# acg-team/ProGraphMSA

Hardware: AMD Instinct MI355X
Metric: DP cell-updates/sec (GCUPS) + wall-clock on 256 seqs × 1000 aa, WAG (higher is better)
Workload: dtype f32

## Files before the change

include/pgm_hip.h:

```cpp
#ifndef PGM_HIP_H_
#define PGM_HIP_H_

#include <stdint.h>
#include <stddef.h>

#ifdef __cplusplus
extern "C" {
#endif

#define PGM_OK 0
#define PGM_ERR_INVALID 1
#define PGM_ERR_DEVICE 2
#define PGM_ERR_BACKTRACK 3
#define PGM_ERR_NOMEM 4

#define PGM_GAP 0xFFFFFFFFu


typedef struct pgm_graph {
    uint32_t n;
    uint32_t dim;
    const double *sites;
    const int32_t *e_rowptr;
    const uint32_t *e_col;
// ... 61 lines not shown
uint64_t pgm_align_batch_cells(const pgm_align_batch *b);
int pgm_align_batch_time(pgm_ctx *ctx, pgm_align_batch *b, int reps, float *ms_prep,
                         float *ms_emission, float *ms_fill, float *ms_traceback);
int pgm_align_batch_stage_times(pgm_align_batch *b, int reset, float *ms_prep, float *ms_emission, float *ms_fill,
                                uint32_t *launches);
int pgm_align_batch_job_times(pgm_ctx *ctx, pgm_align_batch *b, uint64_t *ticks);
int pgm_align_batch_test_stall(pgm_align_batch *b, uint32_t job, uint32_t band, uint32_t spin_limit);
int pgm_test_cu_shares(uint32_t cus, double lean_cost, uint32_t nlean, double band_cost, uint32_t nbands, double rest_cost,
                       uint32_t nrest, uint32_t ncrit, double longest_chain, uint32_t *out4);
#define PGM_PLAN_HEAD 23
#define PGM_PLAN_DHEAD 9
#define PGM_PLAN_JOB 19
int pgm_test_batch_plan(uint32_t njobs, const pgm_graph *const *g1, const pgm_graph *const *g2, const pgm_model *const *model,
                        const pgm_scores *scores, uint32_t flags, const pgm_site_ref *res1, const pgm_site_ref *res2, uint32_t cus,
                        uint32_t *head, double *dhead, uint32_t *job_fields, uint32_t *items, uint32_t *bands, uint32_t *lean_list, int32_t *tblist);
int pgm_align_batch_read_matrices(pgm_ctx *ctx, pgm_align_batch *b, uint32_t job, float *M,
                                  float *X, float *Y, float *W, float *S);

int pgm_nw_pairs_batch(pgm_ctx *ctx, uint32_t dim, const int32_t *score, int32_t gap_open,
                       int32_t gap_extend, uint32_t nseq, const int8_t *syms,
                       const uint32_t *offs, uint32_t npairs, const uint32_t *pi,
                       const uint32_t *pj, int32_t *counts, uint32_t *gaps);
#define PGM_NW_REDUCED 1u
int pgm_nw_pairs_submit(pgm_ctx *ctx, uint32_t dim, const int32_t *score, int32_t gap_open,
                        int32_t gap_extend, uint32_t nseq, const int8_t *syms,
                        const uint32_t *offs, uint32_t npairs, const uint32_t *pi,
                        const uint32_t *pj, uint32_t flags, int32_t *counts, uint32_t *gaps, int *ticket);
int pgm_nw_pairs_wait(pgm_ctx *ctx, int ticket);
float pgm_nw_last_kernel_ms(pgm_ctx *ctx);
void *pgm_host_alloc(size_t bytes);
// ... 144 lines not shown
```

prographmsa_amd/__init__.py:

```python
import ctypes as C
import os

_HERE = os.path.dirname(os.path.abspath(__file__))
LIB_PATH = os.path.join(_HERE, "lib", "libpgm_hip.so")
PGMSA_PATH = os.path.join(_HERE, "bin", "pgmsa")

PGM_OK, PGM_ERR_INVALID, PGM_ERR_DEVICE, PGM_ERR_BACKTRACK, PGM_ERR_NOMEM = 0, 1, 2, 3, 4
PGM_GAP = 0xFFFFFFFF
PGM_BATCH_KEEP_MATRICES = 1
PGM_NW_REDUCED = 1
PGM_MERGE_RESIDENT = 1


class pgm_graph(C.Structure):
    _fields_ = [("n", C.c_uint32), ("dim", C.c_uint32), ("sites", C.POINTER(C.c_double)),
                ("e_rowptr", C.POINTER(C.c_int32)), ("e_col", C.POINTER(C.c_uint32)), ("e_val", C.POINTER(C.c_float)),
                ("r_rowptr", C.POINTER(C.c_int32)), ("r_col", C.POINTER(C.c_uint32)), ("r_units", C.POINTER(C.c_uint32))]


class pgm_model(C.Structure):
    _fields_ = [("M", C.POINTER(C.c_double)), ("pi", C.POINTER(C.c_double))]


class pgm_scores(C.Structure):
# ... 34 lines not shown
    _fields_ = [("index1", C.c_uint32), ("index2", C.c_uint32), ("dist1", C.c_double), ("dist2", C.c_double)]


class pgm_bionj_pair(C.Structure):
    _fields_ = [("index1", C.c_uint32), ("index2", C.c_uint32)]


class pgm_align_out(C.Structure):
    _fields_ = [("score", C.c_float), ("n_tr_indels", C.c_uint32), ("len", C.c_uint32), ("status", C.c_int32),
                ("map1", C.POINTER(C.c_uint32)), ("map2", C.POINTER(C.c_uint32))]


EXPORTS = [
    "pgm_device_count", "pgm_ctx_create", "pgm_ctx_destroy", "pgm_last_error", "pgm_ctx_device_info",
    "pgm_align_graphs_batch", "pgm_align_batch_create", "pgm_align_batch_create_ex", "pgm_align_batch_create_res", "pgm_align_graphs_batch_res", "pgm_align_batch_run", "pgm_align_batch_fetch",
    "pgm_align_batch_destroy", "pgm_align_batch_cells", "pgm_align_batch_test_stall", "pgm_test_cu_shares", "pgm_test_batch_plan", "pgm_align_batch_stage_times", "pgm_align_batch_job_times", "pgm_align_batch_time", "pgm_align_batch_read_matrices",
    "pgm_nw_pairs_batch", "pgm_nw_pairs_submit", "pgm_nw_pairs_wait", "pgm_nw_last_kernel_ms", "pgm_host_alloc", "pgm_host_free", "pgm_csprofile_load", "pgm_csprofile_create_batch", "pgm_csprofile_create_batch_res",
    "pgm_csprofile_last_kernel_ms", "pgm_mldist_batch", "pgm_prealigned_counts_batch", "pgm_kmer_cosine", "pgm_dist_last_kernel_ms",
    "pgm_kmer_cosine_multi", "pgm_prealigned_counts_multi", "pgm_prealigned_counts_resampled",
    "pgm_merge_profiles_batch", "pgm_merge_profiles_batch_ex", "pgm_resident_reset", "pgm_resident_onehot", "pgm_resident_import", "pgm_merge_last_kernel_ms",
    "pgm_gapmask_extend_batch", "pgm_gap_parsimony_batch", "pgm_parsimony_last_kernel_ms",
    "pgm_wls_load", "pgm_wls_pair_sums_batch", "pgm_wls_last_kernel_ms", "pgm_wls_last_launches",
    "pgm_bionj", "pgm_bionj_multi", "pgm_bionj_last_launches", "pgm_bionj_last_kernel_ms",
    "pgm_bionj_plan", "pgm_bionj_plan_multi",
    "pgm_msa_agreement", "pgm_agreement_last_kernel_ms",
    "pgm_transfer_min", "pgm_transfer_last_kernel_ms", "pgm_transfer_taxa",
    "pgm_tree_likelihood", "pgm_treelik_last_kernel_ms", "pgm_tree_likelihood_rates", "pgm_tree_ancestral", "pgm_tree_nni",
    "pgm_resampled_sums", "pgm_resample_last_kernel_ms",
]


# ... 11 lines not shown
        "pgm_last_error": (C.c_char_p, []),
        "pgm_ctx_device_info": (C.c_int, [vp, C.c_char_p, C.c_size_t, C.POINTER(C.c_int)]),
        "pgm_align_graphs_batch": (C.c_int, [vp, u32, PG, PG, PM, C.POINTER(pgm_scores), C.POINTER(pgm_align_out)]),
        "pgm_align_batch_create": (C.c_int, [vp, u32, PG, PG, PM, C.POINTER(pgm_scores), C.POINTER(vp)]),
        "pgm_align_batch_create_ex": (C.c_int, [vp, u32, PG, PG, PM, C.POINTER(pgm_scores), u32, C.POINTER(vp)]),
        "pgm_align_batch_create_res": (C.c_int, [vp, u32, PG, PG, PM, C.POINTER(pgm_scores), u32, C.POINTER(pgm_site_ref), C.POINTER(pgm_site_ref), C.POINTER(vp)]),
        "pgm_align_graphs_batch_res": (C.c_int, [vp, u32, PG, PG, PM, C.POINTER(pgm_scores), C.POINTER(pgm_site_ref), C.POINTER(pgm_site_ref), C.POINTER(pgm_align_out)]),
        "pgm_align_batch_run": (C.c_int, [vp, vp]),
        "pgm_align_batch_fetch": (C.c_int, [vp, vp, C.POINTER(pgm_align_out)]),
        "pgm_align_batch_destroy": (None, [vp, vp]),
        "pgm_align_batch_cells": (C.c_uint64, [vp]),
        "pgm_align_batch_test_stall": (C.c_int, [vp, u32, u32, u32]),
        "pgm_test_cu_shares": (C.c_int, [u32, C.c_double, u32, C.c_double, u32, C.c_double, u32, u32, C.c_double, C.POINTER(C.c_uint32)]),
        "pgm_test_batch_plan": (C.c_int, [u32, PG, PG, PM, C.POINTER(pgm_scores), u32, C.POINTER(pgm_site_ref), C.POINTER(pgm_site_ref), u32,
                                          C.POINTER(u32), C.POINTER(C.c_double)] + [C.POINTER(u32)] * 4 + [C.POINTER(i32)]),
        "pgm_align_batch_stage_times": (C.c_int, [vp, C.c_int] + [C.POINTER(C.c_float)] * 3 + [C.POINTER(u32)]),
        "pgm_align_batch_job_times": (C.c_int, [vp, vp, C.POINTER(C.c_uint64)]),
        "pgm_align_batch_time": (C.c_int, [vp, vp, C.c_int] + [C.POINTER(C.c_float)] * 4),
        "pgm_align_batch_read_matrices": (C.c_int, [vp, vp, u32] + [C.POINTER(C.c_float)] * 5),
        "pgm_nw_pairs_batch": (C.c_int, [vp, u32, C.POINTER(i32), i32, i32, u32, C.POINTER(C.c_int8), C.POINTER(u32), u32,
                                         C.POINTER(u32), C.POINTER(u32), C.POINTER(i32), C.POINTER(u32)]),
        "pgm_nw_pairs_submit": (C.c_int, [vp, u32, C.POINTER(i32), i32, i32, u32, C.POINTER(C.c_int8), C.POINTER(u32), u32,
                                          C.POINTER(u32), C.POINTER(u32), u32, C.POINTER(i32), C.POINTER(u32), C.POINTER(C.c_int)]),
        "pgm_nw_pairs_wait": (C.c_int, [vp, C.c_int]),
        "pgm_host_alloc": (vp, [C.c_size_t]),
        "pgm_host_free": (None, [vp]),
        "pgm_nw_last_kernel_ms": (C.c_float, [vp]),
        "pgm_csprofile_load": (C.c_int, [vp, u32, u32] + [C.POINTER(C.c_double)] * 3),
        "pgm_csprofile_create_batch": (C.c_int, [vp, u32, C.POINTER(C.c_int8), C.POINTER(u32)] + [C.POINTER(C.c_double)] * 4
                                       + [C.POINTER(C.c_uint64)]),
# ... 253 lines not shown
```

prographmsa_amd/csrc/pgm_align_kernels.h:

```cpp
#ifndef PGM_ALIGN_KERNELS_H_
#define PGM_ALIGN_KERNELS_H_

#include <hip/hip_runtime.h>
#include <math.h>
#include <type_traits>
#include "pgm_device.h"

#define PGM_NEG_INF (-INFINITY)

__device__ __forceinline__ float pgm_ls_log_add(float x, float add) {
    const float a = 2.44247459618085927548717403238913328776812604856113966238617812902399112761292613763080658235564f;
    const float b = -4.2040783745848554315883301529007786406310628696382695994938550046831869207082846248658671f;
    const float c = -0.72123729809042963774358701619456664388406302428056983119308906451199556380646306f;
    const uint32_t bits = __float_as_uint(x);
    const float e = (float)((int32_t)(bits >> 23) - 126);
    const float d = __uint_as_float(((bits << 9) >> 9) ^ 0x3f000000u);
    float t = __fdiv_rn(b, __fsub_rn(d, c));
    const float u = __fadd_rn(e, a);
    t = __fadd_rn(t, add);
    t = __fadd_rn(t, u);
    return t;
}

__device__ __forceinline__ float pgm_emission_finish(float num, float ay, float bx, float match_init) {
    float q = __fdiv_rn(num, __fmul_rn(ay, bx));
    if (q != q) q = __uint_as_float(0xFFC00000u);
    return pgm_ls_log_add(q, match_init);
}

template <int DMAX, int NODES>
__global__ void __launch_bounds__(NODES) pgm_prep_kernel(const PgmJob *__restrict__ jobs, int *__restrict__ sync, uint32_t sync_ints) {
    extern __shared__ float prep_lds[];
    {
        const uint32_t nthreads = gridDim.x * gridDim.y * gridDim.z * NODES;
        const uint32_t gid = ((blockIdx.z * gridDim.y + blockIdx.y) * gridDim.x + blockIdx.x) * NODES + threadIdx.x;
        for (uint32_t i = gid; i < sync_ints; i += nthreads) sync[i] = 0;
    }
    const PgmJob &J = jobs[blockIdx.x];
    const bool first = blockIdx.y == 0;
    const uint32_t n = first ? J.n1 : J.n2;
    const uint32_t v0 = blockIdx.z * NODES;
    if (v0 >= n) return;
    if (J.tabhdr && J.tabhdr[0] == 0) {
        const uint32_t nc = J.dim + 2u;
        bool any = n - 1u >= v0 && n - 1u < v0 + (uint32_t)NODES;
        for (uint32_t c = 0; c < nc; ++c) {
            const uint32_t r = (uint32_t)J.tabhdr[1u + (first ? 0u : nc) + c];
            any = any || (r != 0u && r - 1u >= v0 && r - 1u < v0 + (uint32_t)NODES);
        }
        if (!any) return;
    }
    const uint32_t D = J.dim, DP = J.dp, ST = D + 1;
    float *Mf = prep_lds;
    float *pif = prep_lds + D * D;
    float *nl = pif + D;
    const uint32_t nn = min((uint32_t)NODES, n - v0);
    {
        const int32_t *pp = first ? J.pp1 : J.pp2;
        const uint32_t *pc = first ? J.pc1 : J.pc2, *pu = first ? J.pu1 : J.pu2;
        const float *pv = first ? J.pv1 : J.pv2;
        PgmTbNode *rec = (first ? J.tb1 : J.tb2) + v0;
        for (uint32_t i = threadIdx.x; i < nn * PGM_TB_PK; i += NODES) {
            const uint32_t node = i / PGM_TB_PK, k = i % PGM_TB_PK;
            const int32_t eb = pp[v0 + node];
            const uint32_t cnt = (uint32_t)(pp[v0 + node + 1] - eb);
            const int32_t e = cnt == 0u ? 0 : eb + (int32_t)min(k, cnt - 1u);
// ... 48 lines not shown
        for (uint32_t k = 0; k < D; ++k) {
            float t = 0.0f;
#pragma unroll
            for (int j = 0; j < DMAX; ++j)
                if ((uint32_t)j < D) t = __fadd_rn(t, __fmul_rn(Mf[j + D * k], g[j]));
            nl[v * ST + k] = t;
        }
    }
    __syncthreads();
    for (uint32_t i = threadIdx.x; i < nn * DP; i += NODES) {
        const uint32_t node = i / DP, k = i % DP;
        dst[i] = k < D ? nl[node * ST + k] : 0.0f;
    }
}

#define PGM_TAB_HDR 136
__global__ void __launch_bounds__(256) pgm_classify_kernel(const PgmJob *__restrict__ jobs) {
    const PgmJob &J = jobs[blockIdx.x];
    if (!J.tabhdr) return;
    const bool first = blockIdx.y == 0;
    const uint32_t n = first ? J.n1 : J.n2, D = J.dim;
    const double *sites = first ? J.sites1 : J.sites2;
    const uint32_t *smap = first ? J.smap1 : J.smap2;
    uint8_t *cls = (uint8_t *)(first ? J.cls1 : J.cls2);
    const float uni = (float)(1.0 / (double)D);
    for (uint32_t v = blockIdx.z * blockDim.x + threadIdx.x; v < n; v += gridDim.z * blockDim.x) {
        const double *col = sites + (size_t)D * (smap ? smap[v] : v);
        uint32_t nz = 0, sym = 0;
        bool same = true;
        float vs = 0.f;
        const float g0 = (float)col[0];
// ... 15 lines not shown
__device__ __forceinline__ size_t pgm_cell_index(const PgmJob &J, uint32_t y, uint32_t x) {
    const uint32_t b = y / PGM_ROWS, l = PGM_HALO + (y - b * PGM_ROWS);
    return ((size_t)b * J.tsteps + (x + l)) * 64u + l;
}
__device__ __forceinline__ float4 pgm_load_cell(const PgmJob &J, uint32_t y, uint32_t x) {
    return J.cells[pgm_cell_index(J, y, x)];
}

__device__ __forceinline__ float pgm_dpp_wave_shr1(float src, float lane0_value) {
    return __int_as_float(__builtin_amdgcn_update_dpp(__float_as_int(lane0_value), __float_as_int(src), 0x138, 0xf, 0xf, false));
}

#define PGM_GLOBAL __attribute__((address_space(1)))
typedef float pgm_v4f __attribute__((ext_vector_type(4)));
template <class T> __device__ __forceinline__ T pgm_gld(const T *p) { return *(const PGM_GLOBAL T *)(uintptr_t)p; }
#define PGM_EM_TB 4
template <int DP, int RB>
__global__ void __launch_bounds__(4 * PGM_ROWS) pgm_emission_skew_kernel(const PgmJob *__restrict__ jobs) {
    typedef float pgm_v2f __attribute__((ext_vector_type(2)));
    constexpr int NT = DP / 4;
    constexpr int COLS = 64 + PGM_EM_TB * PGM_BLOCK - PGM_HALO - 1;
    constexpr int STR = DP + 1;
    __shared__ pgm_v2f tp[(COLS + 1) * STR];
    __shared__ float bq[COLS];
    const PgmJob &J = jobs[blockIdx.z];
    const uint32_t tb0 = blockIdx.x * PGM_EM_TB;
    const uint32_t rsh = J.rshift, nvb = J.nb << rsh;
    if (tb0 >= J.nblk || 4u * RB * blockIdx.y >= nvb) return;
    if (J.tabhdr && pgm_gld(J.tabhdr) == 0) return;
    auto row_of = [&](uint32_t v, uint32_t lane_) { return ((((v >> rsh) << 6) + lane_) << rsh) | (v & ((1u << rsh) - 1u)); };
    auto sblock_of = [&](uint32_t v, uint32_t tb_) { return ((((size_t)(v >> rsh) * J.nblk + tb_) << rsh) | (v & ((1u << rsh) - 1u))); };
    const uint32_t t0 = tb0 * PGM_BLOCK;
    const int cbase = (int)t0 - 63;
    if ((DP == 20 || DP == 4) && RB == 1) {
        constexpr int TE = DP + 1;
        float *const tab = (float *)tp;
        static_assert(COLS * TE <= (COLS + 1) * STR * 2, "score table must fit the column staging area");
        static_assert(DP > 20 || TE <= 32, "row classes must fit As");
        __shared__ float As[32];
        const uint32_t fb0 = 4u * blockIdx.y + threadIdx.x / PGM_ROWS;
        const uint32_t fl = threadIdx.x % PGM_ROWS;
        const bool active = fb0 < nvb;
        int sym = DP;
        bool plain = true;
        float a_row = 0.f;
        if (active) {
            const uint32_t y = row_of(fb0, fl);
            const uint32_t yc = (y + 1 < J.n1) ? y : 0u;
            const float4 *src = (const float4 *)(J.g1f + (size_t)DP * yc);
            int nz = 0;
#pragma unroll
            for (int q = 0; q < NT; ++q) {
                const float4 v = src[q];
                const float vv[4] = {v.x, v.y, v.z, v.w};
#pragma unroll
// ... 48 lines not shown
        float4 v = make_float4(0.f, 0.f, 0.f, 0.f);
        if (c >= 0 && c <= (int)J.ncol) v = t2q[(size_t)NT * c + q];
        const float vv[4] = {v.x, v.y, v.z, v.w};
#pragma unroll
        for (int u = 0; u < 4; ++u) {
            const int k = 4 * q + u;
            if (ci < COLS) tpf[2 * (ci * STR + k)] = vv[u];
            if (ci > 0) tpf[2 * ((ci - 1) * STR + k) + 1] = vv[u];
        }
    }
    for (int i = threadIdx.x; i < COLS; i += 4 * PGM_ROWS) {
        const int col = cbase + i;
        bq[i] = (col >= 0 && col <= (int)J.ncol) ? J.b2[col] : 0.f;
    }
    __syncthreads();
    const uint32_t b0 = (4u * blockIdx.y + threadIdx.x / PGM_ROWS) * RB;
    const int l = PGM_HALO + (int)(threadIdx.x % PGM_ROWS);
    if (b0 >= nvb) return;
    float gy[RB][DP], ay[RB];
#pragma unroll
    for (int r = 0; r < RB; ++r) {
        const uint32_t y = row_of(b0 + (uint32_t)r, (uint32_t)(l - PGM_HALO));
        const uint32_t yc = (y + 1 < J.n1) ? y : 0u;
        const float4 *src = (const float4 *)(J.g1f + (size_t)DP * yc);
#pragma unroll
        for (int q = 0; q < NT; ++q) {
            const float4 v = src[q];
            gy[r][4 * q] = v.x; gy[r][4 * q + 1] = v.y; gy[r][4 * q + 2] = v.z; gy[r][4 * q + 3] = v.w;
        }
        ay[r] = J.a1[yc];
    }
// ... 2301 lines not shown
```

prographmsa_amd/csrc/pgm_capi.hip:

```cpp
#include <hip/hip_runtime.h>

#include <algorithm>
#include <cmath>
#include <cstdio>
#include <thread>
#include <atomic>
#include <chrono>
#include <queue>
#include <cstdlib>
#include <cstring>
#include <numeric>
#include <mutex>
#include <string>
#include <unordered_set>
#include <vector>
#include <sys/mman.h>

#include "pgm_align_kernels.h"
#include "pgm_crit_kernels.h"
#include "pgm_nw_kernels.h"
#include "pgm_csprofile_kernels.h"
#include "pgm_dist_kernels.h"
#include "pgm_merge_kernels.h"
#include "pgm_parsimony_kernels.h"
// ... 137 lines not shown
    size_t in_bytes = 0, work_bytes = 0, cell_bytes = 0, out_bytes = 0, s_bytes = 0, small_bytes = 0;
    size_t cap[8] = {0, 0, 0, 0, 0, 0, 0, 0};
    uint8_t *h_out = nullptr;
    uint8_t *h_in = nullptr;
    int *h_flag = nullptr;
    int *d_sync = nullptr;
    size_t sync_ints = 0;
    uint32_t lq_off = 0;
    PgmJob *d_jobs = nullptr;
    uint32_t *d_order = nullptr;
    PgmItem *d_items = nullptr;
    uint32_t *d_lean = nullptr;
    PgmItem *d_bands = nullptr;
    int2 *d_tblist = nullptr;
    unsigned long long *d_times = nullptr;
    int *d_tabhdr = nullptr;
    hipEvent_t ev_fork = nullptr, ev_join = nullptr;
    hipEvent_t ev_join_b = nullptr, ev_join_c = nullptr;
    uint32_t test_spin_limit = 0, test_stall_job = 0xFFFFFFFFu, test_stall_band = 0;
    double acc_ms[3] = {0, 0, 0};
    uint32_t acc_n = 0;
    bool ev_pending = false;
    std::vector<size_t> res_off, map1_off, map2_off;
    hipEvent_t ev[5] = {nullptr, nullptr, nullptr, nullptr, nullptr};
};
static const struct BatchBuffer { int slot; size_t reserve_mb; uint8_t *pgm_align_batch::*ptr; size_t pgm_align_batch::*bytes; } kBatchBuffers[6] = {
    {pgm_ctx::C_IN, 128, &pgm_align_batch::d_in, &pgm_align_batch::in_bytes}, {pgm_ctx::C_WORK, 256, &pgm_align_batch::d_work, &pgm_align_batch::work_bytes},
    {pgm_ctx::C_CELLS, 2048, &pgm_align_batch::d_cells, &pgm_align_batch::cell_bytes}, {pgm_ctx::C_OUT, 8, &pgm_align_batch::d_out, &pgm_align_batch::out_bytes},
    {pgm_ctx::C_S, 1024, &pgm_align_batch::d_S, &pgm_align_batch::s_bytes}, {pgm_ctx::C_SMALL, 4, &pgm_align_batch::d_small, &pgm_align_batch::small_bytes}};

// ... 228 lines not shown
}

#define PGM_STATUS_PENDING 0x7ffffff0
struct PrepTier { uint32_t tier, threads; size_t lds; };
static PrepTier prep_tier(uint32_t maxdim) {
    const uint32_t tier = alphabet_tier(maxdim), threads = tier == 64u ? 64u : 256u;
    return {tier, threads, ((size_t)maxdim * maxdim + maxdim + threads * ((size_t)maxdim + 1)) * sizeof(float)};
}
static hipError_t launch_all(pgm_ctx *ctx, pgm_align_batch *b, bool timed) {
    hipStream_t s = ctx->stream;
    const BatchSchedule &S = b->sched;
    hipError_t e;
    for (uint32_t i = 0; i < b->njobs; ++i) ((PgmJob::Result *)(b->h_out + b->res_off[i]))->status = PGM_STATUS_PENDING;
    if (timed && (e = hipEventRecord(b->ev[0], s)) != hipSuccess) return e;
    const PrepTier T = prep_tier(b->maxdim);
    const dim3 pg(b->njobs, 2, (b->maxn + T.threads - 1) / T.threads);
    if (T.tier == 4) hipLaunchKernelGGL((pgm_prep_kernel<4, 256>), pg, dim3(256), T.lds, s, b->d_jobs, b->d_sync, (uint32_t)b->sync_ints);
    else if (T.tier == 20) hipLaunchKernelGGL((pgm_prep_kernel<20, 256>), pg, dim3(256), T.lds, s, b->d_jobs, b->d_sync, (uint32_t)b->sync_ints);
    else hipLaunchKernelGGL((pgm_prep_kernel<64, 64>), pg, dim3(64), T.lds, s, b->d_jobs, b->d_sync, (uint32_t)b->sync_ints);
    if ((e = hipGetLastError()) != hipSuccess) return e;
    if (timed && (e = hipEventRecord(b->ev[1], s)) != hipSuccess) return e;
    const dim3 eg((b->maxnblk + PGM_EM_TB - 1) / PGM_EM_TB, (b->maxnb + 3) / 4, b->njobs);
    if (T.tier == 4) hipLaunchKernelGGL((pgm_emission_skew_kernel<4, 1>), eg, dim3(4 * PGM_ROWS), 0, s, b->d_jobs);
    else if (T.tier == 20) hipLaunchKernelGGL((pgm_emission_skew_kernel<20, 1>), eg, dim3(4 * PGM_ROWS), 0, s, b->d_jobs);
    else hipLaunchKernelGGL((pgm_emission_skew_kernel<64, 1>), eg, dim3(4 * PGM_ROWS), 0, s, b->d_jobs);
    if ((e = hipGetLastError()) != hipSuccess) return e;
    if (timed && (e = hipEventRecord(b->ev[2], s)) != hipSuccess) return e;
    const uint32_t spin_limit = b->test_spin_limit ? b->test_spin_limit : PGM_SPIN_LIMIT, stall_job = b->test_stall_job, stall_band = b->test_stall_band;
    const bool fork = S.nlean != 0;
    const bool bandk = S.nbands != 0;
    const bool tbk = (S.nitems != 0 || bandk) && (S.ntb + S.ntb_c + S.ntb_b) != 0;
    const bool critk = S.ncrit != 0;
    if ((fork || bandk || critk) && (e = hipEventRecord(b->ev_fork, s)) != hipSuccess) return e;
    if (critk && (e = hipStreamWaitEvent(ctx->stream4, b->ev_fork, 0)) != hipSuccess) return e;
    if (fork && (e = hipStreamWaitEvent(ctx->stream2, b->ev_fork, 0)) != hipSuccess) return e;
    if (bandk && (e = hipStreamWaitEvent(ctx->stream3, b->ev_fork, 0)) != hipSuccess) return e;
    const uint32_t nrest = S.nitems - S.ncrit;
    hipStream_t sc = critk ? s : ctx->stream4, sr = critk ? ctx->stream4 : s;
    auto sweep = [&](hipStream_t st, uint32_t workers, const PgmItem *list, uint32_t n, bool c3, uint32_t ticket_off) {
        if (c3) hipLaunchKernelGGL(pgm_crit_kernel, dim3(workers), dim3(64 * PGM_C3_WAVES), 0, st, b->d_jobs, list, n, b->d_sync, spin_limit, stall_job, stall_band, ticket_off);
// ... 21 lines not shown
        if (tbk && S.ntb_c) tracebacks(sc, S.ncrit_workers, S.ntb, S.ntb_c, b->lq_off + 2 * njp, 16u);
        if ((e = hipGetLastError()) != hipSuccess) return e;
    }
    if (tbk && S.ntb) {
        tracebacks(sr, S.ntb_workers, 0u, S.ntb, b->lq_off, 0u);
        if ((e = hipGetLastError()) != hipSuccess) return e;
    }
    if (critk && (e = hipEventRecord(b->ev_join_c, ctx->stream4)) != hipSuccess) return e;
    if (bandk && (e = hipStreamWaitEvent(s, b->ev_join_b, 0)) != hipSuccess) return e;
    if (critk && (e = hipStreamWaitEvent(s, b->ev_join_c, 0)) != hipSuccess) return e;
    if (fork && ((e = hipEventRecord(b->ev_join, ctx->stream2)) != hipSuccess || (e = hipStreamWaitEvent(s, b->ev_join, 0)) != hipSuccess)) return e;
    if (timed && (e = hipEventRecord(b->ev[3], s)) != hipSuccess) return e;
    if (timed && (e = hipEventRecord(b->ev[4], s)) != hipSuccess) return e;
    return hipSuccess;
}
struct SmallLayout { size_t sync, jobs, order, items, lean, tblist, bands, times, tabhdr, total_bands; bool any_lean; };
static SmallLayout layout_small(pgm_align_batch *b) {
    SmallLayout s;
    const uint32_t njobs = b->njobs;
    s.total_bands = 0; s.any_lean = false;
    for (const PgmJob &J : b->jobs) { s.total_bands += J.nb; s.any_lean = s.any_lean || (J.lean && !J.keep_cells); }
    DevLayout SM;
    s.sync = SM.take(b->sync_ints * sizeof(int)); s.jobs = SM.take(sizeof(PgmJob) * std::max(1u, njobs));
    s.order = SM.take(4 * (size_t)std::max(1u, njobs)); s.items = SM.take(sizeof(PgmItem) * std::max<size_t>(1, s.total_bands));
    s.lean = SM.take(4 * (size_t)std::max(1u, njobs)); s.tblist = SM.take(8 * (size_t)std::max(1u, njobs));
    s.bands = SM.take(sizeof(PgmItem) * std::max<size_t>(1, s.total_bands)); s.times = SM.take(16 * (size_t)std::max(1u, njobs) + 16);
    s.tabhdr = SM.take(s.any_lean ? 4 * (size_t)PGM_TAB_HDR * njobs : 16);
    b->small_bytes = SM.bytes;
    return s;
}

static double now_ms() { return std::chrono::duration<double, std::milli>(std::chrono::steady_clock::now().time_since_epoch()).count(); }

struct BatchAlloc {
    std::atomic<int> state{0};
    hipError_t err = hipSuccess, host_err = hipSuccess;
    uint8_t *h_out_dev = nullptr;
    double ms_dev = 0, ms_host = 0, ms_slot[6] = {0, 0, 0, 0, 0, 0};
};
static void take_batch_buffers(pgm_ctx *ctx, pgm_align_batch *b, SmallLayout sm, BatchAlloc *A) {
    const double ta0 = now_ms();
    hipError_t e2 = hipSetDevice(ctx->device);
// ... 1 lines not shown
    for (int k = 0; k < 6 && e2 == hipSuccess; ++k) {
        const BatchBuffer &s = kBatchBuffers[k];
        e2 = cache_take(ctx, s.slot, b->*s.bytes, (void **)&(b->*s.ptr), &b->cap[s.slot]);
        const double t = now_ms(); A->ms_slot[k] = t - tprev; tprev = t;
    }
    if (e2 == hipSuccess) {
        b->d_sync = (int *)(b->d_small + sm.sync);
        b->d_jobs = (PgmJob *)(b->d_small + sm.jobs);
        b->d_order = (uint32_t *)(b->d_small + sm.order);
        b->d_items = (PgmItem *)(b->d_small + sm.items);
        b->d_lean = (uint32_t *)(b->d_small + sm.lean);
        b->d_tblist = (int2 *)(b->d_small + sm.tblist);
        b->d_bands = (PgmItem *)(b->d_small + sm.bands);
        b->d_times = (unsigned long long *)(b->d_small + sm.times);
        b->d_tabhdr = sm.any_lean ? (int *)(b->d_small + sm.tabhdr) : nullptr;
    }
    A->err = e2;
    A->state.store(e2 == hipSuccess ? 1 : -1, std::memory_order_release);
    A->ms_dev = now_ms() - ta0;
    if (e2 == hipSuccess) {
        hipError_t e3 = cache_take(ctx, pgm_ctx::C_HOST, b->out_bytes + 64, (void **)&b->h_out, &b->cap[pgm_ctx::C_HOST]);
        if (e3 == hipSuccess) b->h_flag = (int *)(b->h_out + (b->out_bytes + 15) / 16 * 16);
        if (e3 == hipSuccess) e3 = hipHostGetDevicePointer((void **)&A->h_out_dev, b->h_out, 0);
        A->host_err = e3;
    }
    A->ms_host = now_ms() - ta0 - A->ms_dev;
}

struct CreateGuard {
    pgm_ctx *ctx;
// ... 80 lines not shown
                                       S.nworkers, S.nlean_workers, S.nband_workers, S.nwide_workers, S.ncrit_workers, S.ntb_workers, S.ntb_b_workers,
                                       S.crit_c3, S.rest_c3, S.capacity, (uint32_t)S.total_b, (uint32_t)S.total, (uint32_t)S.total_c};
    const double d[PGM_PLAN_DHEAD] = {S.rsweep, S.t_goal, S.lean_cost, S.band_cost, S.band_end, S.other_cost, S.fill_end, S.crit_end, Z.pro.longest_crit_chain};
    memcpy(head, h, sizeof h);
    memcpy(dhead, d, sizeof d);
    for (uint32_t i = 0; i < njobs; ++i) {
        const PgmJob &J = jobs[i];
        const uint32_t f[PGM_PLAN_JOB] = {J.lean, J.has_extras, J.mode2, J.hD, J.hDX, J.slot_bytes, J.aux_off, J.ov_off, J.rh_off, J.c3_off, J.nov2, J.has_far, J.long1, J.long2,
                                          J.crit3, J.far_slack, J.nslots, Z.off[i].s1.ngeneric + Z.off[i].s2.ngeneric, Z.off[i].s1.nkill + Z.off[i].s2.nkill};
        memcpy(job_fields + (size_t)PGM_PLAN_JOB * i, f, sizeof f);
    }
    if (S.nitems) memcpy(items, S.items.data(), sizeof(PgmItem) * S.nitems);
    if (S.nbands) memcpy(bands, S.bands.data(), sizeof(PgmItem) * S.nbands);
    if (S.nlean) memcpy(lean_list, S.lean_list.data(), 4 * (size_t)S.nlean);
    if (S.ntb + S.ntb_c + S.ntb_b) memcpy(tblist, S.tblist.data(), 8 * (size_t)(S.ntb + S.ntb_c + S.ntb_b));
    return PGM_OK;
}

int pgm_align_batch_create(pgm_ctx *ctx, uint32_t njobs, const pgm_graph *const *g1, const pgm_graph *const *g2,
                           const pgm_model *const *model, const pgm_scores *scores, pgm_align_batch **out) {
    return pgm_align_batch_create_ex(ctx, njobs, g1, g2, model, scores, 0u, out);
}

int pgm_align_batch_create_ex(pgm_ctx *ctx, uint32_t njobs, const pgm_graph *const *g1, const pgm_graph *const *g2,
                              const pgm_model *const *model, const pgm_scores *scores, uint32_t flags, pgm_align_batch **out) {
    return pgm_align_batch_create_res(ctx, njobs, g1, g2, model, scores, flags, nullptr, nullptr, out);
}

int pgm_align_batch_create_res(pgm_ctx *ctx, uint32_t njobs, const pgm_graph *const *g1, const pgm_graph *const *g2,
                               const pgm_model *const *model, const pgm_scores *scores, uint32_t flags,
// ... 59 lines not shown
    b->order = size_order(b->jobs);
    b->sched = plan_schedule(b->jobs, b->order, cus);
    const BatchSchedule &S = b->sched;
    if (cprof && njobs)
        fprintf(stderr, "    work lists: longest chain of sweeps %.0f us, goal %.0f us; lean %zu jobs %.0f us-worker on %u CUs; bands %zu, %.0f us-worker on %u CUs (simulated end %.0f us); items %zu, %.0f us-worker on %u CUs (simulated end %.0f us), of the longest chains %zu on %u CUs (%.0f us)\n",
                S.rsweep, S.t_goal, (size_t)S.nlean, S.lean_cost, S.nlean_workers, S.total_b, S.band_cost, S.nband_workers, S.band_end, S.total, S.other_cost, S.capacity, S.fill_end, S.total_c, S.ncrit_workers, S.crit_end);
    const double tc4 = now_ms();
    if (S.nitems > std::max<size_t>(1, sm.total_bands)) return fail(PGM_ERR_DEVICE, "work list longer than the number of bands");
    if ((e = (hipError_t)upload_err.load()) != hipSuccess ||
        (e = hipMemcpyAsync(b->d_tblist, S.tblist.data(), 8 * S.tblist.size(), hipMemcpyHostToDevice, ctx->stream)) != hipSuccess ||
        (e = hipMemcpyAsync(b->d_jobs, b->jobs.data(), sizeof(PgmJob) * njobs, hipMemcpyHostToDevice, ctx->stream)) != hipSuccess ||
        (e = hipMemcpyAsync(b->d_order, b->order.data(), 4 * (size_t)njobs, hipMemcpyHostToDevice, ctx->stream)) != hipSuccess ||
        (e = hipMemcpyAsync(b->d_items, S.items.data(), sizeof(PgmItem) * S.items.size(), hipMemcpyHostToDevice, ctx->stream)) != hipSuccess ||
        (e = hipMemcpyAsync(b->d_lean, S.lean_list.data(), 4 * S.lean_list.size(), hipMemcpyHostToDevice, ctx->stream)) != hipSuccess ||
        (e = hipMemcpyAsync(b->d_bands, S.bands.data(), sizeof(PgmItem) * S.bands.size(), hipMemcpyHostToDevice, ctx->stream)) != hipSuccess ||
        (e = classify_lean_jobs(ctx, b)) != hipSuccess ||
        (e = hipStreamSynchronize(ctx->stream)) != hipSuccess)
        return fail(PGM_ERR_DEVICE, std::string("upload: ") + hipGetErrorString(e));
    for (int k = 0; k < 5; ++k) (void)hipEventCreate(&b->ev[k]);
    (void)hipEventCreateWithFlags(&b->ev_fork, hipEventDisableTiming);
    (void)hipEventCreateWithFlags(&b->ev_join, hipEventDisableTiming);
    (void)hipEventCreateWithFlags(&b->ev_join_b, hipEventDisableTiming);
    (void)hipEventCreateWithFlags(&b->ev_join_c, hipEventDisableTiming);
    if (cprof)
        fprintf(stderr, "    create: sizes %.2f ms, pinned input block %.2f, flatten %.2f, wait for the allocations %.2f (device %.2f, pinned results %.2f), work list %.2f, upload of %.1f MB %.2f\n",
                tc0 - tcs, tc1 - tc0, tc2 - tc1, tc3 - tc2, A.ms_dev, A.ms_host, tc4 - tc3, b->in_bytes / 1e6, now_ms() - tc4);
    if (cprof)
        fprintf(stderr, "    device buffers: inputs %.1f MB %.2f ms, work %.1f MB %.2f, cells %.1f MB %.2f, results %.1f MB %.2f, S %.1f MB %.2f, small %.2f\n",
                b->in_bytes / 1e6, A.ms_slot[0], b->work_bytes / 1e6, A.ms_slot[1], b->cell_bytes / 1e6, A.ms_slot[2], b->out_bytes / 1e6, A.ms_slot[3], b->s_bytes / 1e6, A.ms_slot[4], A.ms_slot[5]);
    *out = G.release();
    return PGM_OK;
// ... 235 lines not shown
```

prographmsa_amd/csrc/pgm_device.h:

```cpp
#ifndef PGM_DEVICE_H_
#define PGM_DEVICE_H_

#include <stdint.h>
#include "../../include/pgm_hip.h"

#define PGM_MAX_DIM 64
#define PGM_HALO 0
#define PGM_ROWS 64
#define PGM_VL 16
#define PGM_BLOCK 8
#define PGM_NRING 128
#define PGM_KF 4
#define PGM_KF8 8
#define PGM_DCAP 28
#define PGM_PF 4
#define PGM_REMOTE_MAX 128
#define PGM_WAVES 8
#define PGM_WIDE_WAVES 4
#define PGM_POOL 163584
#define PGM_CPARTS 3
#define PGM_AUX_RES 0
#define PGM_AUX_SBLK 3072
#define PGM_AUX_EL 9216
#define PGM_AUX_CNT 13312
// ... 109 lines not shown
#define PGM_LK_H 16u
#define PGM_LK_TAB (3u * PGM_LK_T * PGM_LK_T)
__host__ __device__ inline uint32_t pgm_lk_first(uint32_t n1, uint32_t n2, uint32_t lcols, uint32_t r) {
    const uint32_t w = lcols < PGM_LK_W ? lcols : PGM_LK_W;
    const uint64_t xc = ((uint64_t)(PGM_LK_T * r + PGM_LK_T / 2u) * (n2 - 1u)) / (n1 - 1u);
    const uint32_t g = (uint32_t)(xc / PGM_LK_T);
    const uint32_t lo = g >= w / 2u ? g - w / 2u : 0u;
    return lo + w > lcols ? lcols - w : lo;
}

struct PgmItem {
    uint32_t job, band;
    uint32_t prio, count;
};

#endif
```

prographmsa_amd/csrc/pgm_plan.h:

```cpp
#ifndef PGM_PLAN_H_
#define PGM_PLAN_H_

#include <hip/hip_vector_types.h>

#include <algorithm>
#include <cmath>
#include <cstring>
#include <numeric>
#include <queue>
#include <vector>

#include "pgm_device.h"

namespace {

constexpr double kTauChain = 0.45;
constexpr double kTauExtras = 0.65;
constexpr double kTauMode2 = 0.6;
constexpr double kTauCrit = 0.42;
constexpr double kTauLean = 0.34;
constexpr double kEager = 0.7;
constexpr double kLag = PGM_ROWS + 3.0 * PGM_BLOCK;
constexpr double kLagCritEst = 80.0;
constexpr double kLagWideEst = 78.0;
// ... 609 lines not shown
    }
    for (const PgmItem &it : S.bands) group[it.job] = 2;
    uint32_t cnt[3] = {0, 0, 0};
    for (int pass = 0; pass < 3; ++pass)
        for (uint32_t q = 0; q < njobs; ++q) { const uint32_t i = order[q]; if (!jobs[i].lean && group[i] == pass) { S.tblist.push_back(make_int2((int)i, last_item[i])); ++cnt[pass]; } }
    S.ntb = cnt[0]; S.ntb_c = cnt[1]; S.ntb_b = cnt[2];
    const uint32_t all_cus = std::max(1u, cus) - S.nlean_workers;
    S.ntb_workers = std::max(1u, (S.ntb_b || S.ntb_c) ? S.nworkers : all_cus);
    S.ntb_b_workers = std::max(1u, (S.ntb || S.ntb_c) ? S.nband_workers : all_cus);
    if (S.bands.empty()) S.bands.push_back(PgmItem{0u, 0u, 0u, 0u});
    if (S.lean_list.empty()) S.lean_list.push_back(0u);
    if (S.tblist.empty()) S.tblist.push_back(make_int2(0, 0));
    return S;
}

}

#endif
```

Before: 80.80.

## Launch prep and emission kernels over compacted host-built work lists

Replaces the dense 3D grids of the prep and emission kernels with 1D grids indexed into host-built lists of (job, tile) entries. Blocks that would have exited early (beyond a job's size, or skipped because of the lean class table) are no longer launched, and emission tiles are ordered largest job first. This removes idle block-scheduling overhead from mixed-size batches. The cost is an extra device-to-host copy of the class headers plus a stream synchronize during batch creation.

```diff
diff --git a/include/pgm_hip.h b/include/pgm_hip.h
--- a/include/pgm_hip.h
+++ b/include/pgm_hip.h
@@ -99,6 +99,9 @@
 int pgm_test_batch_plan(uint32_t njobs, const pgm_graph *const *g1, const pgm_graph *const *g2, const pgm_model *const *model,
                         const pgm_scores *scores, uint32_t flags, const pgm_site_ref *res1, const pgm_site_ref *res2, uint32_t cus,
                         uint32_t *head, double *dhead, uint32_t *job_fields, uint32_t *items, uint32_t *bands, uint32_t *lean_list, int32_t *tblist);
+int pgm_test_precompute_lists(uint32_t njobs, const pgm_graph *const *g1, const pgm_graph *const *g2, const pgm_model *const *model,
+                              const pgm_scores *scores, uint32_t flags, const int32_t *tabhdr, uint32_t cap_em, uint32_t cap_prep,
+                              uint32_t *info, uint32_t *em, uint32_t *prep);
 int pgm_align_batch_read_matrices(pgm_ctx *ctx, pgm_align_batch *b, uint32_t job, float *M,
                                   float *X, float *Y, float *W, float *S);
 
diff --git a/prographmsa_amd/__init__.py b/prographmsa_amd/__init__.py
--- a/prographmsa_amd/__init__.py
+++ b/prographmsa_amd/__init__.py
@@ -72,7 +72,7 @@
 EXPORTS = [
     "pgm_device_count", "pgm_ctx_create", "pgm_ctx_destroy", "pgm_last_error", "pgm_ctx_device_info",
     "pgm_align_graphs_batch", "pgm_align_batch_create", "pgm_align_batch_create_ex", "pgm_align_batch_create_res", "pgm_align_graphs_batch_res", "pgm_align_batch_run", "pgm_align_batch_fetch",
-    "pgm_align_batch_destroy", "pgm_align_batch_cells", "pgm_align_batch_test_stall", "pgm_test_cu_shares", "pgm_test_batch_plan", "pgm_align_batch_stage_times", "pgm_align_batch_job_times", "pgm_align_batch_time", "pgm_align_batch_read_matrices",
+    "pgm_align_batch_destroy", "pgm_align_batch_cells", "pgm_align_batch_test_stall", "pgm_test_cu_shares", "pgm_test_batch_plan", "pgm_test_precompute_lists", "pgm_align_batch_stage_times", "pgm_align_batch_job_times", "pgm_align_batch_time", "pgm_align_batch_read_matrices",
     "pgm_nw_pairs_batch", "pgm_nw_pairs_submit", "pgm_nw_pairs_wait", "pgm_nw_last_kernel_ms", "pgm_host_alloc", "pgm_host_free", "pgm_csprofile_load", "pgm_csprofile_create_batch", "pgm_csprofile_create_batch_res",
     "pgm_csprofile_last_kernel_ms", "pgm_mldist_batch", "pgm_prealigned_counts_batch", "pgm_kmer_cosine", "pgm_dist_last_kernel_ms",
     "pgm_kmer_cosine_multi", "pgm_prealigned_counts_multi", "pgm_prealigned_counts_resampled",
@@ -114,6 +114,7 @@
         "pgm_test_cu_shares": (C.c_int, [u32, C.c_double, u32, C.c_double, u32, C.c_double, u32, u32, C.c_double, C.POINTER(C.c_uint32)]),
         "pgm_test_batch_plan": (C.c_int, [u32, PG, PG, PM, C.POINTER(pgm_scores), u32, C.POINTER(pgm_site_ref), C.POINTER(pgm_site_ref), u32,
                                           C.POINTER(u32), C.POINTER(C.c_double)] + [C.POINTER(u32)] * 4 + [C.POINTER(i32)]),
+        "pgm_test_precompute_lists": (C.c_int, [u32, PG, PG, PM, C.POINTER(pgm_scores), u32, C.POINTER(i32), u32, u32] + [C.POINTER(u32)] * 3),
         "pgm_align_batch_stage_times": (C.c_int, [vp, C.c_int] + [C.POINTER(C.c_float)] * 3 + [C.POINTER(u32)]),
         "pgm_align_batch_job_times": (C.c_int, [vp, vp, C.POINTER(C.c_uint64)]),
         "pgm_align_batch_time": (C.c_int, [vp, vp, C.c_int] + [C.POINTER(C.c_float)] * 4),
diff --git a/prographmsa_amd/csrc/pgm_align_kernels.h b/prographmsa_amd/csrc/pgm_align_kernels.h
--- a/prographmsa_amd/csrc/pgm_align_kernels.h
+++ b/prographmsa_amd/csrc/pgm_align_kernels.h
@@ -29,27 +29,21 @@
 }
 
 template <int DMAX, int NODES>
-__global__ void __launch_bounds__(NODES) pgm_prep_kernel(const PgmJob *__restrict__ jobs, int *__restrict__ sync, uint32_t sync_ints) {
+__global__ void __launch_bounds__(NODES) pgm_prep_kernel(const PgmJob *__restrict__ jobs, const PgmPrepSlice *__restrict__ slices, uint32_t nslices,
+                                                         int *__restrict__ sync, uint32_t sync_ints) {
     extern __shared__ float prep_lds[];
     {
-        const uint32_t nthreads = gridDim.x * gridDim.y * gridDim.z * NODES;
-        const uint32_t gid = ((blockIdx.z * gridDim.y + blockIdx.y) * gridDim.x + blockIdx.x) * NODES + threadIdx.x;
+        const uint32_t nthreads = gridDim.x * NODES;
+        const uint32_t gid = blockIdx.x * NODES + threadIdx.x;
         for (uint32_t i = gid; i < sync_ints; i += nthreads) sync[i] = 0;
     }
-    const PgmJob &J = jobs[blockIdx.x];
-    const bool first = blockIdx.y == 0;
+    if (blockIdx.x >= nslices) return;
+    const PgmPrepSlice sl = slices[blockIdx.x];
+    const PgmJob &J = jobs[sl.job];
+    const bool first = sl.side == 0;
     const uint32_t n = first ? J.n1 : J.n2;
-    const uint32_t v0 = blockIdx.z * NODES;
+    const uint32_t v0 = sl.slice * NODES;
     if (v0 >= n) return;
-    if (J.tabhdr && J.tabhdr[0] == 0) {
-        const uint32_t nc = J.dim + 2u;
-        bool any = n - 1u >= v0 && n - 1u < v0 + (uint32_t)NODES;
-        for (uint32_t c = 0; c < nc; ++c) {
-            const uint32_t r = (uint32_t)J.tabhdr[1u + (first ? 0u : nc) + c];
-            any = any || (r != 0u && r - 1u >= v0 && r - 1u < v0 + (uint32_t)NODES);
-        }
-        if (!any) return;
-    }
     const uint32_t D = J.dim, DP = J.dp, ST = D + 1;
     float *Mf = prep_lds;
     float *pif = prep_lds + D * D;
@@ -128,7 +122,6 @@
     }
 }
 
-#define PGM_TAB_HDR 136
 __global__ void __launch_bounds__(256) pgm_classify_kernel(const PgmJob *__restrict__ jobs) {
     const PgmJob &J = jobs[blockIdx.x];
     if (!J.tabhdr) return;
@@ -174,20 +167,19 @@
 #define PGM_GLOBAL __attribute__((address_space(1)))
 typedef float pgm_v4f __attribute__((ext_vector_type(4)));
 template <class T> __device__ __forceinline__ T pgm_gld(const T *p) { return *(const PGM_GLOBAL T *)(uintptr_t)p; }
-#define PGM_EM_TB 4
 template <int DP, int RB>
-__global__ void __launch_bounds__(4 * PGM_ROWS) pgm_emission_skew_kernel(const PgmJob *__restrict__ jobs) {
+__global__ void __launch_bounds__(4 * PGM_ROWS) pgm_emission_skew_kernel(const PgmJob *__restrict__ jobs, const PgmEmTile *__restrict__ tiles) {
     typedef float pgm_v2f __attribute__((ext_vector_type(2)));
     constexpr int NT = DP / 4;
     constexpr int COLS = 64 + PGM_EM_TB * PGM_BLOCK - PGM_HALO - 1;
     constexpr int STR = DP + 1;
     __shared__ pgm_v2f tp[(COLS + 1) * STR];
     __shared__ float bq[COLS];
-    const PgmJob &J = jobs[blockIdx.z];
-    const uint32_t tb0 = blockIdx.x * PGM_EM_TB;
+    const PgmEmTile tile = tiles[blockIdx.x];
+    const PgmJob &J = jobs[tile.job];
+    const uint32_t tb0 = tile.tg * PGM_EM_TB, vb0 = 4u * tile.vg;
     const uint32_t rsh = J.rshift, nvb = J.nb << rsh;
-    if (tb0 >= J.nblk || 4u * RB * blockIdx.y >= nvb) return;
-    if (J.tabhdr && pgm_gld(J.tabhdr) == 0) return;
+    if (tb0 >= J.nblk || RB * vb0 >= nvb) return;
     auto row_of = [&](uint32_t v, uint32_t lane_) { return ((((v >> rsh) << 6) + lane_) << rsh) | (v & ((1u << rsh) - 1u)); };
     auto sblock_of = [&](uint32_t v, uint32_t tb_) { return ((((size_t)(v >> rsh) * J.nblk + tb_) << rsh) | (v & ((1u << rsh) - 1u))); };
     const uint32_t t0 = tb0 * PGM_BLOCK;
@@ -198,7 +190,7 @@
         static_assert(COLS * TE <= (COLS + 1) * STR * 2, "score table must fit the column staging area");
         static_assert(DP > 20 || TE <= 32, "row classes must fit As");
         __shared__ float As[32];
-        const uint32_t fb0 = 4u * blockIdx.y + threadIdx.x / PGM_ROWS;
+        const uint32_t fb0 = vb0 + threadIdx.x / PGM_ROWS;
         const uint32_t fl = threadIdx.x % PGM_ROWS;
         const bool active = fb0 < nvb;
         int sym = DP;
@@ -277,7 +269,7 @@
         bq[i] = (col >= 0 && col <= (int)J.ncol) ? J.b2[col] : 0.f;
     }
     __syncthreads();
-    const uint32_t b0 = (4u * blockIdx.y + threadIdx.x / PGM_ROWS) * RB;
+    const uint32_t b0 = (vb0 + threadIdx.x / PGM_ROWS) * RB;
     const int l = PGM_HALO + (int)(threadIdx.x % PGM_ROWS);
     if (b0 >= nvb) return;
     float gy[RB][DP], ay[RB];
diff --git a/prographmsa_amd/csrc/pgm_capi.hip b/prographmsa_amd/csrc/pgm_capi.hip
--- a/prographmsa_amd/csrc/pgm_capi.hip
+++ b/prographmsa_amd/csrc/pgm_capi.hip
@@ -175,6 +175,10 @@
     PgmItem *d_bands = nullptr;
     int2 *d_tblist = nullptr;
     unsigned long long *d_times = nullptr;
+    PgmEmTile *d_emtiles = nullptr;
+    PgmPrepSlice *d_prepslices = nullptr;
+    uint32_t nemtiles = 0, nprepslices = 0;
+    PrecomputeLists pre;
     int *d_tabhdr = nullptr;
     hipEvent_t ev_fork = nullptr, ev_join = nullptr;
     hipEvent_t ev_join_b = nullptr, ev_join_c = nullptr;
@@ -433,16 +437,17 @@
     for (uint32_t i = 0; i < b->njobs; ++i) ((PgmJob::Result *)(b->h_out + b->res_off[i]))->status = PGM_STATUS_PENDING;
     if (timed && (e = hipEventRecord(b->ev[0], s)) != hipSuccess) return e;
     const PrepTier T = prep_tier(b->maxdim);
-    const dim3 pg(b->njobs, 2, (b->maxn + T.threads - 1) / T.threads);
-    if (T.tier == 4) hipLaunchKernelGGL((pgm_prep_kernel<4, 256>), pg, dim3(256), T.lds, s, b->d_jobs, b->d_sync, (uint32_t)b->sync_ints);
-    else if (T.tier == 20) hipLaunchKernelGGL((pgm_prep_kernel<20, 256>), pg, dim3(256), T.lds, s, b->d_jobs, b->d_sync, (uint32_t)b->sync_ints);
-    else hipLaunchKernelGGL((pgm_prep_kernel<64, 64>), pg, dim3(64), T.lds, s, b->d_jobs, b->d_sync, (uint32_t)b->sync_ints);
+    const dim3 pg(std::max(1u, b->nprepslices));
+    if (T.tier == 4) hipLaunchKernelGGL((pgm_prep_kernel<4, 256>), pg, dim3(256), T.lds, s, b->d_jobs, b->d_prepslices, b->nprepslices, b->d_sync, (uint32_t)b->sync_ints);
+    else if (T.tier == 20) hipLaunchKernelGGL((pgm_prep_kernel<20, 256>), pg, dim3(256), T.lds, s, b->d_jobs, b->d_prepslices, b->nprepslices, b->d_sync, (uint32_t)b->sync_ints);
+    else hipLaunchKernelGGL((pgm_prep_kernel<64, 64>), pg, dim3(64), T.lds, s, b->d_jobs, b->d_prepslices, b->nprepslices, b->d_sync, (uint32_t)b->sync_ints);
     if ((e = hipGetLastError()) != hipSuccess) return e;
     if (timed && (e = hipEventRecord(b->ev[1], s)) != hipSuccess) return e;
-    const dim3 eg((b->maxnblk + PGM_EM_TB - 1) / PGM_EM_TB, (b->maxnb + 3) / 4, b->njobs);
-    if (T.tier == 4) hipLaunchKernelGGL((pgm_emission_skew_kernel<4, 1>), eg, dim3(4 * PGM_ROWS), 0, s, b->d_jobs);
-    else if (T.tier == 20) hipLaunchKernelGGL((pgm_emission_skew_kernel<20, 1>), eg, dim3(4 * PGM_ROWS), 0, s, b->d_jobs);
-    else hipLaunchKernelGGL((pgm_emission_skew_kernel<64, 1>), eg, dim3(4 * PGM_ROWS), 0, s, b->d_jobs);
+    const dim3 eg(b->nemtiles);
+    if (b->nemtiles == 0) {}
+    else if (T.tier == 4) hipLaunchKernelGGL((pgm_emission_skew_kernel<4, 1>), eg, dim3(4 * PGM_ROWS), 0, s, b->d_jobs, b->d_emtiles);
+    else if (T.tier == 20) hipLaunchKernelGGL((pgm_emission_skew_kernel<20, 1>), eg, dim3(4 * PGM_ROWS), 0, s, b->d_jobs, b->d_emtiles);
+    else hipLaunchKernelGGL((pgm_emission_skew_kernel<64, 1>), eg, dim3(4 * PGM_ROWS), 0, s, b->d_jobs, b->d_emtiles);
     if ((e = hipGetLastError()) != hipSuccess) return e;
     if (timed && (e = hipEventRecord(b->ev[2], s)) != hipSuccess) return e;
     const uint32_t spin_limit = b->test_spin_limit ? b->test_spin_limit : PGM_SPIN_LIMIT, stall_job = b->test_stall_job, stall_band = b->test_stall_band;
@@ -494,7 +499,7 @@
     if (timed && (e = hipEventRecord(b->ev[4], s)) != hipSuccess) return e;
     return hipSuccess;
 }
-struct SmallLayout { size_t sync, jobs, order, items, lean, tblist, bands, times, tabhdr, total_bands; bool any_lean; };
+struct SmallLayout { size_t sync, jobs, order, items, lean, tblist, bands, times, tabhdr, emtiles, prepslices, total_bands; bool any_lean; };
 static SmallLayout layout_small(pgm_align_batch *b) {
     SmallLayout s;
     const uint32_t njobs = b->njobs;
@@ -506,6 +511,10 @@
     s.lean = SM.take(4 * (size_t)std::max(1u, njobs)); s.tblist = SM.take(8 * (size_t)std::max(1u, njobs));
     s.bands = SM.take(sizeof(PgmItem) * std::max<size_t>(1, s.total_bands)); s.times = SM.take(16 * (size_t)std::max(1u, njobs) + 16);
     s.tabhdr = SM.take(s.any_lean ? 4 * (size_t)PGM_TAB_HDR * njobs : 16);
+    size_t ntiles = 0, nslices = 0;
+    const uint32_t nodes = prep_slice_nodes(b->maxdim);
+    for (const PgmJob &J : b->jobs) { ntiles += em_tiles_of(J); nslices += prep_slices_of(J, nodes); }
+    s.emtiles = SM.take(sizeof(PgmEmTile) * std::max<size_t>(1, ntiles)); s.prepslices = SM.take(sizeof(PgmPrepSlice) * std::max<size_t>(1, nslices));
     b->small_bytes = SM.bytes;
     return s;
 }
@@ -537,6 +546,8 @@
         b->d_bands = (PgmItem *)(b->d_small + sm.bands);
         b->d_times = (unsigned long long *)(b->d_small + sm.times);
         b->d_tabhdr = sm.any_lean ? (int *)(b->d_small + sm.tabhdr) : nullptr;
+        b->d_emtiles = (PgmEmTile *)(b->d_small + sm.emtiles);
+        b->d_prepslices = (PgmPrepSlice *)(b->d_small + sm.prepslices);
     }
     A->err = e2;
     A->state.store(e2 == hipSuccess ? 1 : -1, std::memory_order_release);
@@ -647,6 +658,26 @@
     if (S.nbands) memcpy(bands, S.bands.data(), sizeof(PgmItem) * S.nbands);
     if (S.nlean) memcpy(lean_list, S.lean_list.data(), 4 * (size_t)S.nlean);
     if (S.ntb + S.ntb_c + S.ntb_b) memcpy(tblist, S.tblist.data(), 8 * (size_t)(S.ntb + S.ntb_c + S.ntb_b));
+    return PGM_OK;
+}
+
+int pgm_test_precompute_lists(uint32_t njobs, const pgm_graph *const *g1, const pgm_graph *const *g2, const pgm_model *const *model,
+                              const pgm_scores *scores, uint32_t flags, const int32_t *tabhdr, uint32_t cap_em, uint32_t cap_prep,
+                              uint32_t *info, uint32_t *em, uint32_t *prep) {
+    if (!info || (cap_em && !em) || (cap_prep && !prep) || (njobs && (!g1 || !g2 || !model || !scores))) return fail(PGM_ERR_INVALID, "null argument");
+    std::vector<char> two_chains(njobs, 0);
+    for (uint32_t i = 0; i < njobs; ++i) two_chains[i] = job_is_two_chains(g1[i], g2[i]) ? 1 : 0;
+    std::vector<PgmJob> jobs;
+    BatchSizes Z;
+    const int invalid = plan_sizes(njobs, g1, g2, model, scores, flags, nullptr, nullptr, two_chains, 256u, jobs, Z);
+    if (invalid >= 0) return fail(PGM_ERR_INVALID, "invalid job " + std::to_string(invalid));
+    const uint32_t nodes = prep_slice_nodes(Z.maxdim);
+    const PrecomputeLists P = plan_precompute(jobs, tabhdr, nodes);
+    info[0] = alphabet_tier(Z.maxdim); info[1] = nodes; info[2] = PGM_EM_TB; info[3] = (uint32_t)P.em.size(); info[4] = (uint32_t)P.prep.size();
+    if (P.em.size() > cap_em || P.prep.size() > cap_prep) return fail(PGM_ERR_INVALID, "precompute lists longer than the caller's arrays");
+    static_assert(sizeof(PgmEmTile) == 12 && sizeof(PgmPrepSlice) == 12, "three words per list entry");
+    if (!P.em.empty()) memcpy(em, P.em.data(), sizeof(PgmEmTile) * P.em.size());
+    if (!P.prep.empty()) memcpy(prep, P.prep.data(), sizeof(PgmPrepSlice) * P.prep.size());
     return PGM_OK;
 }
 
@@ -736,7 +767,16 @@
         (e = hipMemcpyAsync(b->d_items, S.items.data(), sizeof(PgmItem) * S.items.size(), hipMemcpyHostToDevice, ctx->stream)) != hipSuccess ||
         (e = hipMemcpyAsync(b->d_lean, S.lean_list.data(), 4 * S.lean_list.size(), hipMemcpyHostToDevice, ctx->stream)) != hipSuccess ||
         (e = hipMemcpyAsync(b->d_bands, S.bands.data(), sizeof(PgmItem) * S.bands.size(), hipMemcpyHostToDevice, ctx->stream)) != hipSuccess ||
-        (e = classify_lean_jobs(ctx, b)) != hipSuccess ||
+        (e = classify_lean_jobs(ctx, b)) != hipSuccess)
+        return fail(PGM_ERR_DEVICE, std::string("upload: ") + hipGetErrorString(e));
+    std::vector<int> tabhdr(b->d_tabhdr ? (size_t)PGM_TAB_HDR * njobs : 0);
+    if ((!tabhdr.empty() && (e = hipMemcpyAsync(tabhdr.data(), b->d_tabhdr, 4 * tabhdr.size(), hipMemcpyDeviceToHost, ctx->stream)) != hipSuccess) ||
+        (e = hipStreamSynchronize(ctx->stream)) != hipSuccess)
+        return fail(PGM_ERR_DEVICE, std::string("upload: ") + hipGetErrorString(e));
+    b->pre = plan_precompute(b->jobs, tabhdr.empty() ? nullptr : tabhdr.data(), prep_slice_nodes(b->maxdim));
+    b->nemtiles = (uint32_t)b->pre.em.size(); b->nprepslices = (uint32_t)b->pre.prep.size();
+    if ((b->nemtiles && (e = hipMemcpyAsync(b->d_emtiles, b->pre.em.data(), sizeof(PgmEmTile) * b->pre.em.size(), hipMemcpyHostToDevice, ctx->stream)) != hipSuccess) ||
+        (b->nprepslices && (e = hipMemcpyAsync(b->d_prepslices, b->pre.prep.data(), sizeof(PgmPrepSlice) * b->pre.prep.size(), hipMemcpyHostToDevice, ctx->stream)) != hipSuccess) ||
         (e = hipStreamSynchronize(ctx->stream)) != hipSuccess)
         return fail(PGM_ERR_DEVICE, std::string("upload: ") + hipGetErrorString(e));
     for (int k = 0; k < 5; ++k) (void)hipEventCreate(&b->ev[k]);
diff --git a/prographmsa_amd/csrc/pgm_device.h b/prographmsa_amd/csrc/pgm_device.h
--- a/prographmsa_amd/csrc/pgm_device.h
+++ b/prographmsa_amd/csrc/pgm_device.h
@@ -147,4 +147,9 @@
     uint32_t prio, count;
 };
 
+#define PGM_EM_TB 4
+#define PGM_TAB_HDR 136
+struct PgmEmTile { uint32_t job, vg, tg; };
+struct PgmPrepSlice { uint32_t job, side, slice; };
+
 #endif
diff --git a/prographmsa_amd/csrc/pgm_plan.h b/prographmsa_amd/csrc/pgm_plan.h
--- a/prographmsa_amd/csrc/pgm_plan.h
+++ b/prographmsa_amd/csrc/pgm_plan.h
@@ -647,6 +647,49 @@
     return S;
 }
 
+struct PrecomputeLists {
+    std::vector<PgmEmTile> em;
+    std::vector<PgmPrepSlice> prep;
+};
+inline uint32_t prep_slice_nodes(uint32_t maxdim) { return alphabet_tier(maxdim) == 64u ? 64u : 256u; }
+inline bool job_has_class_header(const PgmJob &J) { return J.lean && !J.keep_cells; }
+inline uint32_t em_tiles_of(const PgmJob &J) { return (((J.nb << J.rshift) + 3u) / 4u) * ((J.nblk + PGM_EM_TB - 1u) / PGM_EM_TB); }
+inline uint32_t prep_slices_of(const PgmJob &J, uint32_t nodes) { return (J.n1 + nodes - 1u) / nodes + (J.n2 + nodes - 1u) / nodes; }
+static PrecomputeLists plan_precompute(const std::vector<PgmJob> &jobs, const int *tabhdr, uint32_t nodes) {
+    PrecomputeLists P;
+    const uint32_t njobs = (uint32_t)jobs.size();
+    auto header = [&](uint32_t i) { return (tabhdr && job_has_class_header(jobs[i])) ? tabhdr + (size_t)PGM_TAB_HDR * i : nullptr; };
+    auto from_table = [&](uint32_t i) { const int *h = header(i); return h && h[0] == 0; };
+    std::vector<uint32_t> order(njobs);
+    std::iota(order.begin(), order.end(), 0u);
+    std::stable_sort(order.begin(), order.end(), [&](uint32_t x, uint32_t y) { return em_tiles_of(jobs[x]) > em_tiles_of(jobs[y]); });
+    for (uint32_t i : order) {
+        if (from_table(i)) continue;
+        const PgmJob &J = jobs[i];
+        const uint32_t nvg = ((J.nb << J.rshift) + 3u) / 4u, ntg = (J.nblk + PGM_EM_TB - 1u) / PGM_EM_TB;
+        for (uint32_t vg = 0; vg < nvg; ++vg)
+            for (uint32_t tg = 0; tg < ntg; ++tg) P.em.push_back(PgmEmTile{i, vg, tg});
+    }
+    for (uint32_t i = 0; i < njobs; ++i) {
+        const PgmJob &J = jobs[i];
+        const bool table = from_table(i);
+        const int *h = header(i);
+        for (uint32_t side = 0; side < 2u; ++side) {
+            const uint32_t n = side == 0 ? J.n1 : J.n2, nc = J.dim + 2u;
+            for (uint32_t sl = 0; sl * nodes < n; ++sl) {
+                const uint32_t v0 = sl * nodes;
+                bool any = !table || (n - 1u >= v0 && n - 1u - v0 < nodes);
+                for (uint32_t c = 0; !any && c < nc; ++c) {
+                    const uint32_t r = (uint32_t)h[1u + side * nc + c];
+                    any = r != 0u && r - 1u >= v0 && r - 1u - v0 < nodes;
+                }
+                if (any) P.prep.push_back(PgmPrepSlice{i, side, sl});
+            }
+        }
+    }
+    return P;
+}
+
 }
 
 #endif
```

Measured after the change: 80.54. Within noise of the previous version (-0.3%).
